# haoheliu/AudioLDM2

Measured on AMD Instinct MI355X. Metric: audio_seconds_per_second, higher is better.
Workload: dtype f32 storage/accumulate; each product = 6 bf16 MFMA partial products of exact 3-part operand splits (fp32-grade); 1 GPU; audioldm2-full: batch 8 prompts/GPU x 1 GPU, 10.24 s @16 kHz, 200 DDIM steps, CFG 3.5, eta 1.0, n_candidates 1; one step = sample_log + VAE decode + HiFi-GAN + D2H of the waveform; synthetic conditioning, random-init weights, host-CPU RNG noise; global_batch=8, parallelism=prompt-sharded replicas x1, weight_broadcast_bytes=0

## Files before the change

### audioldm2_amd/csrc/api.hip

```cpp
#include "common.h"
#include <string.h>

namespace aldm {
static thread_local char g_err[512] = "";
void set_error(const char* fmt, ...) {
    va_list ap;
    va_start(ap, fmt);
    vsnprintf(g_err, sizeof(g_err), fmt, ap);
    va_end(ap);
}
}

extern "C" int aldm_version(void) { return 25; }
extern "C" const char* aldm_last_error(void) { return aldm::g_err; }
```

### audioldm2_amd/csrc/igemm.hip

```cpp
#include "igemm_kernel.h"
#include <algorithm>
#include <atomic>
#include <stdlib.h>

namespace aldm {

int igemm_launch_pre0(int BM, int BN, int kgroups, bool uni, bool w8, dim3 grid, hipStream_t st, const IgemmK& p);
int igemm_launch_pre1(int BM, int BN, int kgroups, bool uni, bool w8, dim3 grid, hipStream_t st, const IgemmK& p);
int igemm_launch_pre2(int BM, int BN, int kgroups, bool uni, bool w8, dim3 grid, hipStream_t st, const IgemmK& p);
int igemm_launch_pre3(int BM, int BN, int kgroups, bool uni, bool w8, dim3 grid, hipStream_t st, const IgemmK& p);
int igemm_launch_pre4(int BM, int BN, int kgroups, bool uni, bool w8, dim3 grid, hipStream_t st, const IgemmK& p);
int igemm_launch_bx_pre0(int BM, int BN, int kgroups, bool uni, bool w8, dim3 grid, hipStream_t st, const IgemmK& p);
int igemm_launch_bx_pre1(int BM, int BN, int kgroups, bool uni, bool w8, dim3 grid, hipStream_t st, const IgemmK& p);
int igemm_launch_bx_pre2(int BM, int BN, int kgroups, bool uni, bool w8, dim3 grid, hipStream_t st, const IgemmK& p);
int igemm_launch_bx_pre3(int BM, int BN, int kgroups, bool uni, bool w8, dim3 grid, hipStream_t st, const IgemmK& p);

int igemm_launch_dma(int BM, int BN, int nst, int parts, bool f16, dim3 grid, hipStream_t st, const IgemmK& p);
bool igemm_dma_config_ok(int BM, int BN, int nst, int parts);
#ifdef ALDM_TEST_HOOKS
extern std::atomic<int> g_debug_drop_product;
#endif
int igemm_launch_dma_ws(int BM, int BN, int nst, int parts, int blocks, hipStream_t st, const IgemmK& p);
bool igemm_dma_ws_config_ok(int BM, int BN, int nst, int parts);
int igemm_dma_ws_blocks_per_cu(int BM, int BN, int nst, int parts);
// ... 22 lines not shown
    f32x4 v = *reinterpret_cast<const f32x4*>(w);
    int s = 1;
    for (; s + 3 < p.splits; s += 4) {
        const f32x4 a0 = *reinterpret_cast<const f32x4*>(w + (int64_t)s * slab);
        const f32x4 a1 = *reinterpret_cast<const f32x4*>(w + (int64_t)(s + 1) * slab);
        const f32x4 a2 = *reinterpret_cast<const f32x4*>(w + (int64_t)(s + 2) * slab);
        const f32x4 a3 = *reinterpret_cast<const f32x4*>(w + (int64_t)(s + 3) * slab);
        v += a0;
        v += a1;
        v += a2;
        v += a3;
    }
    for (; s < p.splits; ++s) v += *reinterpret_cast<const f32x4*>(w + (int64_t)s * slab);
    const int b = m / p.OHW;
    int64_t orow = m;
    if (d.out_mul > 0) {
        const int qq = m - b * p.OHW;
        const int t = qq * d.out_mul + d.out_off;
        if ((unsigned)t >= (unsigned)d.out_len) return;
        orow = (int64_t)b * d.out_len + t;
    }
    float* outp = d.out ? d.out + (int64_t)z * d.stride_o : nullptr;
    const float* resp = d.res ? d.res + (int64_t)z * d.stride_o : nullptr;
    const int64_t o = orow * d.ldo + n;
    f32x4 r;
#pragma unroll
    for (int j = 0; j < 4; ++j) r[j] = epi_value(d, p.rb_ld, outp, resp, b, o + j, n + j, v[j]);
    if (outp) {
#pragma unroll
        for (int j = 0; j < 4; ++j) outp[o + j] = r[j];
    }
    if (d.out_split) {
        if (d.out_split_act == ALDM_ACT_LRELU) {
#pragma unroll
            for (int j = 0; j < 4; ++j) r[j] = r[j] > 0.0f ? r[j] : r[j] * d.out_split_slope;
        }
// ... 3 lines not shown

__global__ void pack_weight_kernel(const float* __restrict__ src, float* __restrict__ dst, int N,
                                   int Cin, int KH, int KW, int Kg, int Npad) {
    const int64_t total = (int64_t)Kg * Npad * 4;
    for (int64_t i = blockIdx.x * (int64_t)blockDim.x + threadIdx.x; i < total;
         i += (int64_t)gridDim.x * blockDim.x) {
        const int j = i & 3;
        const int n = (i >> 2) % Npad;
        const int kg = (i >> 2) / Npad;
        const int k = kg * 4 + j;
        float v = 0.f;
        if (n < N && k < KH * KW * Cin) {
            const int tap = k / Cin, ci = k - tap * Cin;
            const int kh = tap / KW, kw = tap - kh * KW;
            v = src[(((int64_t)n * Cin + ci) * KH + kh) * KW + kw];
        }
        dst[i] = v;
    }
}

__global__ void pack_weight_tr_kernel(const float* __restrict__ src, float* __restrict__ dst, int N,
                                      int Cin, int KWfull, int T, int phase, int stride, int Kg,
                                      int Npad) {
    const int64_t total = (int64_t)Kg * Npad * 4;
    for (int64_t i = blockIdx.x * (int64_t)blockDim.x + threadIdx.x; i < total;
         i += (int64_t)gridDim.x * blockDim.x) {
        const int jj = i & 3;
        const int n = (i >> 2) % Npad;
        const int kg = (i >> 2) / Npad;
        const int k = kg * 4 + jj;
// ... 249 lines not shown
    ALDM_CHECK(d.SH > 0 && d.SW > 0 && d.DH > 0 && d.DW > 0, "aldm_igemm: bad stride/dilation");
    p.shh = log2_exact(d.up_h);
    p.shw = log2_exact(d.up_w);
    ALDM_CHECK(p.shh >= 0 && p.shw >= 0, "aldm_igemm: upsample factors must be powers of two");
    ALDM_CHECK((reinterpret_cast<uintptr_t>(d.x1) & 15) == 0 &&
                   (reinterpret_cast<uintptr_t>(d.w) & 15) == 0 &&
                   (d.x2 == nullptr || (reinterpret_cast<uintptr_t>(d.x2) & 15) == 0),
               "aldm_igemm: operands must be 16-byte aligned");
    if (d.b_mode == ALDM_B_NT) {
        ALDM_CHECK(d.ldb % 4 == 0 && d.ldb >= d.K, "aldm_igemm: NT ldb=%d invalid", d.ldb);
        p.Npad = d.N;
    } else {
        p.Npad = (d.N + 31) / 32 * 32;
        ALDM_CHECK(d.ldb == 0 || d.ldb == p.Npad, "aldm_igemm: packed ldb must equal Npad");
    }
    if (d.out_mul > 0) ALDM_CHECK(d.OH == 1, "aldm_igemm: row remap requires OH == 1");
    ALDM_CHECK((d.pre_scale == nullptr) == (d.pre_shift == nullptr),
               "aldm_igemm: pre_scale/pre_shift must come together");
    ALDM_CHECK(d.pre_scale == nullptr ||
                   ((reinterpret_cast<uintptr_t>(d.pre_scale) | reinterpret_cast<uintptr_t>(d.pre_shift)) & 15) == 0,
               "aldm_igemm: pre_scale/pre_shift must be 16-byte aligned");
    const bool geglu = d.epi_mode == ALDM_EPI_GEGLU;
    const bool qkv = d.epi_mode == ALDM_EPI_QKV;
    ALDM_CHECK(d.epi_mode == ALDM_EPI_PLAIN || geglu || qkv, "aldm_igemm: unknown epi_mode %d", d.epi_mode);
    if (qkv) {
        auto al16 = [](const void* q) { return (reinterpret_cast<uintptr_t>(q) & 15) == 0; };
        ALDM_CHECK(d.a_split && d.qkv_c > 0 && d.qkv_c % 64 == 0 && d.N == 3 * d.qkv_c && d.qkv_rows > 0 && d.qkv_rows % 32 == 0 &&
                       (((int64_t)d.B * d.OH * d.OW) % d.qkv_rows == 0 ||
                        d.qkv_rows == (((int64_t)d.B * d.OH * d.OW + 31) & ~(int64_t)31)) && d.out && d.k_split && d.vt_split && al16(d.out) &&
                       al16(d.k_split) && al16(d.vt_split) && d.ldo >= d.qkv_c && (d.ldo & 3) == 0 && !d.bias && !d.rowbias &&
                       !d.res && !d.out_split && !d.accumulate && d.out_mul == 0 && d.act == ALDM_ACT_NONE && d.alpha == 1.0f &&
// ... 35 lines not shown
        ALDM_CHECK(d.out_split_c > 0 && d.out_split_c % 32 == 0 && d.out_split_c >= (geglu ? d.N / 2 : d.N) &&
                       d.N % 4 == 0 && d.batch == 1 && (reinterpret_cast<uintptr_t>(d.out_split) & 15) == 0 &&
                       ((reinterpret_cast<uintptr_t>(d.out) | reinterpret_cast<uintptr_t>(d.res)) & 15) == 0 &&
                       (d.out == nullptr || (d.ldo & 3) == 0),
                   "aldm_igemm: out_split needs out_split_c %% 32 == 0 and >= N, N %% 4 == 0, batch 1, aligned out/res");
        ALDM_CHECK(d.out != nullptr || !d.accumulate, "aldm_igemm: accumulate needs an fp32 output");
    }
    if (d.a_split) {
        ALDM_CHECK(d.w_split != nullptr && d.b_mode == ALDM_B_PACKED && d.stride_w == 0 && d.batch == 1,
                   "aldm_igemm: a_split needs packed, split weights and batch 1");
        ALDM_CHECK(d.C2 == 0 && d.C1 % 32 == 0 && pre == PRE_NONE,
                   "aldm_igemm: a_split needs one source with C1 %% 32 == 0 and no prologue (C1=%d C2=%d)", d.C1, d.C2);
        ALDM_CHECK(((reinterpret_cast<uintptr_t>(d.a_split) | reinterpret_cast<uintptr_t>(d.w_split)) & 15) == 0,
                   "aldm_igemm: split images must be 16-byte aligned");
        ALDM_CHECK((int64_t)d.B * d.H * d.W * p.Cin * 2 * d.split_parts < (1ll << 40), "aldm_igemm: split image too large");
        const bool can_split = d.N % 4 == 0 && nk >= 8 && !geglu && !qkv;
        const bool have_ws = d.ws != nullptr && (reinterpret_cast<uintptr_t>(d.ws) & 15) == 0;
        auto dma_cost = [&](int bm, int bn, int nst, int sp, int* sp_eff) -> double {
            const int kt = cdiv(nk, sp);
            sp = cdiv(nk, kt);
            *sp_eff = sp;
            const double blocks = (double)cdiv64(Mz, bm) * cdiv(d.N, bn) * sp;
            const int lds = nst * (bm + bn) * 64 * d.split_parts;
            const int o = std::min(2, (160 * 1024) / lds);
            const double tile_c = (bm / 64) * (bn / 64) * 64.0 * (d.split_parts == 3 ? 6 : 3);
            const double dma_c = (bm + bn) * 64.0 * d.split_parts / 56.0;
            const double L = kt * std::max(tile_c, dma_c);
            const double one = kt * std::max(tile_c + 200.0, dma_c) + 6000.0;
            const int64_t nb = (int64_t)((blocks + 255.0) / 256.0);
            const int64_t full = nb / o, last = nb - full * o;
            double T = full * std::max(one, o * L);
            if (last) T += std::max(one, last * L);
            if (sp > 1) T += 10000.0 + (double)(sp + 1) * Mz * d.N * 4.0 / 2000.0;
            return T;
        };
        int splits = 1, nst = 0;
        const bool hint_fits = d.hint_bm > 0 && (!qkv || (d.hint_bn > 0 && d.qkv_c % d.hint_bn == 0)) && (!geglu || d.hint_bn == 128);
// ... 118 lines not shown
        p.tiles_n = cdiv(d.N, BN);
        p.kt_per_split = cdiv(nk, splits);
        splits = cdiv(nk, p.kt_per_split);
        if (splits > 1 && (!have_ws || d.ws_floats < (int64_t)splits * p.M * d.N)) {
            splits = 1;
            p.kt_per_split = nk;
        }
        p.splits = splits;
        p.kgroups = 1;
        p.bx = 1;
        p.pre = pre;
        p.dma = 1;
        p.nst = nst;
        p.ws = 0;
        p.ws_blocks = 0;
        if (lw_nst > 0) {
            ALDM_CHECK(igemm_dma_lw_config_ok(BM, BN, lw_nst, d.split_parts), "aldm_igemm: no loader-wave DMA kernel for tile %dx%d, %d stages", BM, BN, lw_nst);
            p.ws = 2;
            p.nst = lw_nst;
        }
        if (ws_nst > 0) {
            if (splits == 1 && d.a_fmt == ALDM_FMT_BF16 && d.out_split_parts == d.split_parts && d.out_split_fmt == ALDM_FMT_BF16 &&
                igemm_dma_ws_config_ok(BM, BN, ws_nst, d.split_parts) && dma_ws_eligible(p, BM, BN)) {
                const int ntiles = p.tiles_m * p.tiles_n;
                const int per = cdiv(ntiles, device_cus() * igemm_dma_ws_blocks_per_cu(BM, BN, ws_nst, d.split_parts));
                p.ws = 1;
                p.nst = ws_nst;
                p.ws_blocks = cdiv(ntiles, per);
            } else {
                ALDM_CHECK(!g_force_bm, "aldm_igemm: the persistent DMA kernel cannot run this launch (tile %dx%d, %d stages)", BM,
// ... 93 lines not shown
    p.splits = splits;
    p.kgroups = kgroups;
    p.bx = bx_ok && BN != 32 ? 1 : 0;
    p.pre = pre;
    return 0;
}

extern "C" int aldm_igemm_plan(const aldm_igemm_desc* dd, int* bm, int* bn, int64_t* flops, int* splits,
                               int* kgroups, int* mma) {
    IgemmK p;
    int BM, BN;
    const int rc = igemm_prepare(dd, p, BM, BN);
    if (rc) return rc;
    if (bm) *bm = BM;
    if (bn) *bn = BN;
    if (flops) *flops = 2ll * p.M * p.d.N * p.d.K * p.d.batch;
    if (splits) *splits = p.splits;
    if (kgroups) *kgroups = p.kgroups;
    if (mma) *mma = p.bx ? ALDM_MMA_BF16X6 : ALDM_MMA_F32;
    return 0;
}

extern "C" int aldm_igemm_plan_stages(const aldm_igemm_desc* dd) {
    IgemmK p;
    int BM, BN;
    if (igemm_prepare(dd, p, BM, BN)) return -1;
    if (p.dma && p.ws == 4) return 400 + (BM == 128 && p.ws_blocks == 4 ? 10 : 0) + p.nst;
    return p.dma ? p.nst + 100 * p.ws : 0;
}

extern "C" int aldm_igemm_plan_epilogue(const aldm_igemm_desc* dd) {
// ... 9 lines not shown
    t.ws = reinterpret_cast<float*>(uintptr_t(16));
    t.ws_floats = INT64_MAX;
    IgemmK p;
    int BM, BN;
    if (igemm_prepare(&t, p, BM, BN)) return 0;
    return p.splits > 1 ? (int64_t)p.d.batch * p.splits * p.M * p.d.N : 0;
}

extern "C" int aldm_igemm(const aldm_igemm_desc* dd, void* stream) {
    IgemmK p;
    int BM, BN;
    int rc = igemm_prepare(dd, p, BM, BN);
    if (rc) return rc;
    p.epi_form = plan_epilogue_form(p, BM, BN);
    const aldm_igemm_desc& d = p.d;
    dim3 grid((unsigned)(p.tiles_m * p.tiles_n), (unsigned)p.splits, (unsigned)d.batch);
    hipStream_t st = (hipStream_t)stream;
    const int pre = p.pre;
    const bool uni = p.OHW % BM == 0;
    const int env_w8 = g_wave8_mask < 0 ? default_wave8_mask() : g_wave8_mask;
    const bool gn_pre = pre == PRE_AFFINE || pre == PRE_AFFINE_SILU;
    const int tile_bit = (BM == 128 && BN == 128) ? 1 : (BM == 64 && BN == 128) ? 2 : (BM == 128 && BN == 64) ? 4 : 0;
    const bool w8 = p.kgroups == 1 && d.epi_mode != ALDM_EPI_GEGLU && (env_w8 & tile_bit) != 0 &&
                    (p.bx ? tile_bit == 1 : (gn_pre || (tile_bit == 1 && (env_w8 & 8) != 0)));
#ifdef ALDM_TEST_HOOKS
    if (g_debug_drop_product.load(std::memory_order_relaxed))
        ALDM_CHECK(p.dma && p.ws == 0 && BM == 64 && BN == 128 && p.nst == 2 && d.split_parts == 3,
                   "aldm_igemm: aldm_debug_drop_product is set: force the classic DMA-fed 64x128 tile with 2 stages and 3-part images "
                   "(got dma=%d form=%d tile %dx%d, %d stages, %d parts) or clear the switch", p.dma, p.ws, BM, BN, p.nst, d.split_parts);
#endif
    if (p.dma && p.ws == 4) {
// ... 93 lines not shown
    } else {
        ALDM_CHECK(KH == 1 && stride > 0 && phase >= 0 && phase < stride,
                   "aldm_pack_weight: bad transposed args");
        const int T = (KW + stride - 1) / stride;
        const int K = T * Cin;
        const int Kg = (K + 3) / 4;
        const int64_t total = (int64_t)Kg * Npad * 4;
        const int blocks = (int)std::min<int64_t>(cdiv64(total, 256), 4096);
        hipLaunchKernelGGL(pack_weight_tr_kernel, dim3(blocks), dim3(256), 0, st, src, dst, N, Cin,
                           KW, T, phase, stride, Kg, Npad);
    }
    ALDM_LAUNCH_CHECK("aldm_pack_weight");
    return 0;
}

extern "C" int aldm_pack_kn(const float* src, float* dst, int K, int N, int lds, int batch,
                            int64_t stride_src, int64_t stride_dst, void* stream) {
    ALDM_CHECK(src && dst && K > 0 && N > 0 && lds >= N && batch > 0, "aldm_pack_kn: bad args");
    const int Npad = (N + 31) / 32 * 32;
    const int Kg = (K + 3) / 4;
    const int64_t total = (int64_t)Kg * Npad * 4;
    const int blocks = (int)std::min<int64_t>(cdiv64(total, 256), 4096);
    hipLaunchKernelGGL(pack_kn_kernel, dim3(blocks, batch), dim3(256), 0, (hipStream_t)stream, src,
                       dst, K, N, lds, Kg, Npad, stride_src, stride_dst);
    ALDM_LAUNCH_CHECK("aldm_pack_kn");
    return 0;
}
```

### audioldm2_amd/csrc/igemm_dma.h

```cpp
#pragma once
#include "igemm_epilogue.h"
#include <type_traits>

namespace aldm {

static __device__ __attribute__((aligned(256))) unsigned g_dma_zero_page[256 + 64];

constexpr int dma_stage_slots(int BM, int BN, int NP) { return (BM + BN) * 4 * NP; }
constexpr int dma_lds_bytes(int BM, int BN, int NST, int NP) { return NST * dma_stage_slots(BM, BN, NP) * 16; }
constexpr int dma_blocks_per_cu(int BM, int BN, int NST, int NP) {
    return (160 * 1024) / dma_lds_bytes(BM, BN, NST, NP) >= 2 ? 2 : 1;
}

template <bool F16>
__device__ __forceinline__ f32x16 mfma_32x32x16(const bf16x8 a, const bf16x8 b, const f32x16 c) {
    if constexpr (F16)
        return __builtin_amdgcn_mfma_f32_32x32x16_f16(__builtin_bit_cast(f16x8, a), __builtin_bit_cast(f16x8, b), c, 0, 0, 0);
    else
        return __builtin_amdgcn_mfma_f32_32x32x16_bf16(a, b, c, 0, 0, 0);
}
template <bool F16, int MT, int NT>
__device__ __forceinline__ void unscale_acc(f32x16 (&acc)[MT][NT], float acc_scale) {
    if constexpr (F16) {
#pragma unroll
// ... 53 lines not shown
        tile_m = logical / p.tiles_n;
    }
    const int m0 = tile_m * BM, n0 = tile_n * BN;
    const int split = blockIdx.y;
    const int nk_all = d.K >> 5;
    const int kt0 = split * p.kt_per_split;
    const int kt1 = min(nk_all, kt0 + p.kt_per_split);
#if ALDM_DMA_ABLATE & 32
    const int nk = min(kt1 - kt0, 1);
#else
    const int nk = kt1 - kt0;
#endif

    const char* zero = reinterpret_cast<const char*>(g_dma_zero_page);
    const char* abase = reinterpret_cast<const char*>(d.a_split);
    const char* wbase = reinterpret_cast<const char*>(d.w_split);
    const int cpb = p.Cin >> 5;
    const int taps = d.KH * d.KW;
    const int64_t rowbytes = (int64_t)cpb * PB;

    const int lane_off = ((lane & 3) ^ ((lane >> 4) & 3)) * 16;
    int a_pix[RA], a_h[RA], a_w[RA];
#pragma unroll
    for (int i = 0; i < RA; ++i) {
        const int m = m0 + (wave * RA + i) * 16 + (lane >> 2);
        if (m < p.M) {
            const int b = m / p.OHW;
            const int rem = m - b * p.OHW;
            const int oh = rem / d.OW;
            const int ow = rem - oh * d.OW;
            a_pix[i] = b * d.H;
            a_h[i] = oh * d.SH - d.PH;
            a_w[i] = ow * d.SW - d.PW;
        } else {
            a_pix[i] = 0;
            a_h[i] = -(1 << 28);
            a_w[i] = 0;
        }
    }
    const char* a_ptr[RA];
    int a_step[RA];
    int t_kh, t_kw, t_cb;
    auto set_tap = [&]() {
        const int dh = t_kh * d.DH, dw = t_kw * d.DW;
        const int cboff = t_cb * PB + lane_off;
#pragma unroll
        for (int i = 0; i < RA; ++i) {
            const int ihv = a_h[i] + dh, iwv = a_w[i] + dw;
// ... 203 lines not shown
#if ALDM_DMA_ABLATE & 16
    if (p.M == -12345) {
#pragma unroll
        for (int i = 0; i < MT; ++i)
#pragma unroll
            for (int j = 0; j < NT; ++j)
#pragma unroll
                for (int e = 0; e < 16; ++e) d.ws[(i * NT + j) * 16 + e + threadIdx.x * 256] = acc[i][j][e];
    }
    return;
#endif
    unscale_acc<F16>(acc, d.acc_scale);
    if constexpr (FORM != ALDM_EPI_FORM_GENERIC)
        igemm_epilogue_form<MT, NT, NP, FORM>(p, acc, epre, reinterpret_cast<float*>(&smem[0]), m0, n0, wave, wm, wn, lane);
    else
        igemm_epilogue<MT, NT>(p, acc, reinterpret_cast<float*>(&smem[0]), m0, n0, wave, wm, wn, lane, 0, split);
}

}
```

### audioldm2_amd/csrc/igemm_epilogue.h

```cpp
#pragma once
#include "common.h"

#ifndef ALDM_DMA_ABLATE
#define ALDM_DMA_ABLATE 0
#endif

namespace aldm {

struct IgemmK {
    aldm_igemm_desc d;
    int Cin, M, OHW, HV, WV, shh, shw, Kg, Npad, tiles_m, tiles_n;
    int splits, kt_per_split;
    int kgroups;
    int rb_ld;
    int bx;
    int pre;
    int dma;
    int nst;
    int ws;
    int ws_blocks;
    int os_rows;
    int epi_form;
};

// ... 111 lines not shown
}
__device__ __forceinline__ void split_store4_out(const aldm_igemm_desc& d, void* img, int64_t row, int Cs, int c, const f32x4 v) {
    if (d.out_split_fmt == ALDM_FMT_F16) split_store4_f16(img, row, Cs, c, v, d.out_split_scale);
    else split_store4(img, row, Cs, c, v, d.out_split_parts);
}

template <int P>
__device__ __forceinline__ void split_store4_t(void* img, int64_t row, int Cs, int c, const f32x4 v) {
    static_assert(P == 2 || P == 3, "2 or 3 parts");
    u32x2 part[3];
    if constexpr (P == 2) split4_rn2(v, part);
    else split4(v, part);
    char* base = reinterpret_cast<char*>(img) + (row * (Cs >> 5) + (c >> 5)) * (64 * P) + (c & 31) * 2;
#pragma unroll
    for (int q = 0; q < P; ++q) *reinterpret_cast<u32x2*>(base + q * 64) = part[q];
}

__device__ __forceinline__ float epi_value(const aldm_igemm_desc& d, int rb_ld, const float* __restrict__ outp,
                                           const float* __restrict__ resp, int b, int64_t o, int n, float v) {
    if (d.bias) v += d.bias[n];
    if (d.rowbias) v += d.rowbias[(int64_t)b * rb_ld + n];
    v = act_apply(v, d.act, d.act_slope);
    if (resp) v += resp[o];
    v *= d.alpha;
    if (d.accumulate) v += outp[o];
    return v;
}

__device__ __forceinline__ float silu_fast(float v) {
    return v * __frcp_rn(1.0f + __expf(-v));
// ... 138 lines not shown
        f32x4 v[ITC];
        int64_t rowoff[ITC];
        int64_t srow[ITC];
        int rboff[ITC];
        unsigned okmask = 0;
#pragma unroll
        for (int it = 0; it < ITC; ++it) {
            const int r = (itc + it) * RPI + sr;
            v[it] = *reinterpret_cast<const f32x4*>(&stg[r * SP + sc]);
            const int m = m0 + (wm * MT + i) * 32 + r;
            bool ok = m < p.M && ncol < d.N;
            int b = 0;
            int64_t orow = m;
            if (need_b) {
                b = m / p.OHW;
                if (d.out_mul > 0) {
                    const int qq = m - b * p.OHW;
                    const int t = qq * d.out_mul + d.out_off;
                    ok = ok && (unsigned)t < (unsigned)d.out_len;
                    orow = (int64_t)b * d.out_len + t;
                }
            }
            rowoff[it] = ok ? orow * ld_out + (ncol - col_shift) : 0;
            srow[it] = orow;
            rboff[it] = ok ? b * p.rb_ld + ncol : 0;
            okmask |= ((ok && epi_st) ? 1u : 0u) << it;
        }
        if (split_out) {
#pragma unroll
            for (int it = 0; it < ITC; ++it)
                if ((okmask >> it) & 1u) *reinterpret_cast<f32x4*>(outp + rowoff[it]) = v[it];
            continue;
        }
#pragma unroll
        for (int it = 0; it < ITC; ++it) v[it] += bias4;
        if (d.rowbias) {
// ... 181 lines not shown
```

### audioldm2_amd/lib.py

```python
from __future__ import annotations

import ctypes as C
import os

_HERE = os.path.dirname(os.path.abspath(__file__))
LIB_PATH = os.environ.get("ALDM_LIB_PATH") or os.path.join(_HERE, "libaldm_hip.so")
ABI_VERSION = 25

ACT_NONE, ACT_SILU, ACT_LRELU, ACT_TANH, ACT_LOGCLAMP, ACT_GELU, ACT_GELU_TANH = range(7)
B_PACKED, B_NT = 0, 1
EPI_PLAIN, EPI_GEGLU, EPI_QKV = 0, 1, 2
GN_CHUNKED, GN_FUSED, GN_FUSED_SPLIT = 0, 1, 2
FMT_BF16, FMT_F16 = 0, 1
EPI_FORM_GENERIC, EPI_FORM_PLAIN, EPI_FORM_ROWBIAS, EPI_FORM_RES = range(4)


class IgemmDesc(C.Structure):

    _fields_ = [
        ("x1", C.c_void_p), ("x2", C.c_void_p),
        ("C1", C.c_int32), ("C2", C.c_int32),
        ("pix1", C.c_int32), ("pix2", C.c_int32),
        ("B", C.c_int32), ("H", C.c_int32), ("W", C.c_int32),
        ("up_h", C.c_int32), ("up_w", C.c_int32),
# ... 8 lines not shown
        ("bias", C.c_void_p), ("rowbias", C.c_void_p), ("res", C.c_void_p), ("out", C.c_void_p),
        ("ldo", C.c_int32), ("act", C.c_int32), ("act_slope", C.c_float), ("alpha", C.c_float),
        ("accumulate", C.c_int32),
        ("out_mul", C.c_int32), ("out_off", C.c_int32), ("out_len", C.c_int32),
        ("batch", C.c_int32),
        ("stride_x", C.c_int64), ("stride_w", C.c_int64), ("stride_o", C.c_int64),
        ("rowbias_ld", C.c_int32), ("epi_mode", C.c_int32),
        ("ws", C.c_void_p), ("ws_floats", C.c_int64),
        ("hint_bm", C.c_int32), ("hint_bn", C.c_int32), ("hint_splits", C.c_int32), ("hint_kgroups", C.c_int32),
        ("w_split", C.c_void_p), ("hint_mma", C.c_int32), ("hint_stages", C.c_int32),
        ("a_split", C.c_void_p), ("out_split", C.c_void_p), ("out_split_c", C.c_int32), ("split_parts", C.c_int32),
        ("out_split_act", C.c_int32), ("out_split_slope", C.c_float),
        ("k_split", C.c_void_p), ("vt_split", C.c_void_p), ("qkv_c", C.c_int32), ("qkv_rows", C.c_int32),
        ("a_fmt", C.c_int32), ("acc_scale", C.c_float), ("out_split_parts", C.c_int32),
        ("out_split_fmt", C.c_int32), ("out_split_scale", C.c_float), ("vt_scale", C.c_float),
    ]


MAX_WINDOWS = 32


class WindowStarts(C.Structure):

    _fields_ = [("n", C.c_int), ("s", C.c_int * MAX_WINDOWS)]


MAX_ROWS = 64


class WindowRows(C.Structure):
# ... 28 lines not shown
    "aldm_split_bytes_parts": (C.c_int64, [C.c_int, C.c_int, C.c_int]),
    "aldm_pack_split_bf16_parts": (C.c_int, [C.c_void_p, C.c_void_p, C.c_int, C.c_int, C.c_int, C.c_void_p]),
    "aldm_pack_split_f16": (C.c_int, [C.c_void_p, C.c_void_p, C.c_int, C.c_int, C.c_float, C.c_void_p]),
    "aldm_split_rows_f16": (C.c_int, [C.c_void_p, C.c_void_p, C.c_int, C.c_int, C.c_int64, C.c_int, C.c_void_p, C.c_void_p,
                                      C.c_int, C.c_float, C.c_void_p, C.c_void_p, C.c_int, C.c_float, C.c_void_p]),
    "aldm_groupnorm_split_f16": (C.c_int, [C.c_void_p, C.c_void_p, C.c_int, C.c_int, C.c_int, C.c_int, C.c_int, C.c_float,
                                           C.c_void_p, C.c_void_p, C.c_int, C.c_void_p, C.c_void_p, C.c_void_p, C.c_void_p,
                                           C.c_void_p, C.c_int, C.c_float, C.c_void_p]),
    "aldm_layernorm_split_f16": (C.c_int, [C.c_void_p, C.c_void_p, C.c_void_p, C.c_int, C.c_int, C.c_void_p, C.c_void_p,
                                           C.c_float, C.c_float, C.c_void_p]),
    "aldm_igemm_mma": (C.c_int, [C.c_int]),
    "aldm_split_bytes": (C.c_int64, [C.c_int, C.c_int]),
    "aldm_pack_split_bf16": (C.c_int, [C.c_void_p, C.c_void_p, C.c_int, C.c_int, C.c_void_p]),
    "aldm_pack_weight": (C.c_int, [C.c_void_p, C.c_void_p, C.c_int, C.c_int, C.c_int, C.c_int,
                                   C.c_int, C.c_int, C.c_int, C.c_void_p]),
    "aldm_pack_kn": (C.c_int, [C.c_void_p, C.c_void_p, C.c_int, C.c_int, C.c_int, C.c_int,
                               C.c_int64, C.c_int64, C.c_void_p]),
    "aldm_groupnorm_stats": (C.c_int, [C.c_void_p, C.c_void_p, C.c_int, C.c_int, C.c_int, C.c_int,
                                       C.c_int, C.c_float, C.c_void_p, C.c_void_p, C.c_void_p,
                                       C.c_void_p, C.c_void_p, C.c_void_p]),
    "aldm_gn_ws_floats": (C.c_int64, [C.c_int, C.c_int, C.c_int, C.c_int]),
    "aldm_groupnorm_plan": (C.c_int, [C.c_int] * 6 + [C.POINTER(C.c_int)] * 9),
    "aldm_groupnorm_split": (C.c_int, [C.c_void_p, C.c_void_p, C.c_int, C.c_int, C.c_int, C.c_int, C.c_int, C.c_float,
                                       C.c_void_p, C.c_void_p, C.c_int, C.c_void_p, C.c_void_p, C.c_void_p, C.c_void_p,
                                       C.c_void_p, C.c_int, C.c_void_p]),
    "aldm_layernorm": (C.c_int, [C.c_void_p, C.c_void_p, C.c_int, C.c_int, C.c_void_p, C.c_void_p,
                                 C.c_float, C.c_void_p]),
    "aldm_attention_mma": (C.c_int, [C.c_int]),
    "aldm_attention_sched": (C.c_int, [C.c_int]),
    "aldm_attention_query_tiles": (C.c_int, [C.c_int, C.c_int, C.c_int]),
# ... 177 lines not shown
```

### audioldm2_amd/ops.py

```python
from __future__ import annotations

import ctypes as C
import json
import os
from dataclasses import dataclass
from typing import List, Optional, Sequence, Tuple

import torch

from . import lib as _l
from .lib import (ACT_GELU, ACT_GELU_TANH, ACT_LOGCLAMP, ACT_LRELU, ACT_NONE, ACT_SILU, ACT_TANH, B_NT, B_PACKED,
                  IgemmDesc)


def _stream() -> int:
    return torch.cuda.current_stream().cuda_stream


def _p(t: Optional[torch.Tensor]):
    return None if t is None else t.data_ptr()


def _chk(t: torch.Tensor, name: str):
    if not (t.is_cuda and t.dtype == torch.float32 and t.is_contiguous()):
# ... 467 lines not shown
def pack_conv(weight: torch.Tensor, bias: Optional[torch.Tensor] = None) -> Packed:
    w = weight.detach().to(device="cuda", dtype=torch.float32).contiguous()
    if w.dim() == 2:
        N, Cin, KH, KW = w.shape[0], w.shape[1], 1, 1
    elif w.dim() == 3:
        N, Cin, KH, KW = w.shape[0], w.shape[1], 1, w.shape[2]
    else:
        N, Cin, KH, KW = w.shape
    K = KH * KW * Cin
    dst = torch.empty(((K + 3) // 4) * _npad(N) * 4, device="cuda", dtype=torch.float32)
    lib = _l.load()
    _l.check(lib.aldm_pack_weight(w.data_ptr(), dst.data_ptr(), N, Cin, KH, KW, 0, 0, 1, _stream()),
             "pack_weight")
    b = None if bias is None else bias.detach().to(device="cuda", dtype=torch.float32).contiguous()
    return Packed(dst, N, Cin, KH, KW, b)


def pack_geglu(weight: torch.Tensor, bias: Optional[torch.Tensor]) -> Packed:
    two_inner = weight.shape[0]
    inner = two_inner // 2
    assert weight.dim() == 2 and two_inner % 64 == 0
    g = torch.arange(inner // 32).view(-1, 1, 1)
    j = torch.arange(2).view(1, -1, 1)
    l = torch.arange(32).view(1, 1, -1)
    perm = (j * inner + g * 32 + l).reshape(-1).to(weight.device)
    pw = pack_conv(weight.detach()[perm], None if bias is None else bias.detach()[perm])
    pw.geglu = True
    return pw


# ... 145 lines not shown
    for ph in range(stride):
        dst = torch.empty(((T * Cin + 3) // 4) * _npad(N) * 4, device="cuda", dtype=torch.float32)
        _l.check(lib.aldm_pack_weight(w.data_ptr(), dst.data_ptr(), N, Cin, 1, KW, 1, ph, stride,
                                      _stream()), "pack_weight(tr)")
        out.append(Packed(dst, N, Cin, 1, T, b))
    return out


def conv(x: torch.Tensor, pw: Packed, *, stride=(1, 1), pad=(0, 0), dil=(1, 1), up=(1, 1),
         x2: Optional[torch.Tensor] = None, out_hw: Optional[Tuple[int, int]] = None,
         pre: Optional[Tuple[torch.Tensor, torch.Tensor]] = None, pre_act: int = ACT_NONE,
         pre_slope: float = 0.0, bias: Optional[torch.Tensor] = None,
         rowbias: Optional[torch.Tensor] = None, res: Optional[torch.Tensor] = None,
         act: int = ACT_NONE, act_slope: float = 0.0, alpha: float = 1.0,
         out: Optional[torch.Tensor] = None, accumulate: bool = False,
         remap: Optional[Tuple[int, int, int]] = None,
         use_pw_bias: bool = True, split_out: Optional[str] = None, split_act: int = ACT_NONE, split_slope: float = 0.0):
    is_split = isinstance(x, SplitT)
    if is_split:
        assert x2 is None and pre is None and pre_act == ACT_NONE, "a pre-split operand takes no prologue"
    else:
        _chk(x, "conv.x")
    B, H, W, C1 = x.shape
    C2 = 0
    if x2 is not None:
        _chk(x2, "conv.x2")
        assert x2.shape[:3] == x.shape[:3]
        C2 = x2.shape[3]
    assert C1 + C2 == pw.Cin, f"channels {C1}+{C2} != packed Cin {pw.Cin}"
    VH, VW = H * up[0], W * up[1]
    if out_hw is None:
        OH = (VH + 2 * pad[0] - dil[0] * (pw.KH - 1) - 1) // stride[0] + 1
        OW = (VW + 2 * pad[1] - dil[1] * (pw.KW - 1) - 1) // stride[1] + 1
    else:
        OH, OW = out_hw
    N = pw.N
    if remap is not None:
        out_mul, out_off, out_len = remap
        oshape = (B, 1, out_len, N)
    else:
        out_mul = out_off = out_len = 0
        oshape = (B, OH, OW, N)
    if split_out == "only":
        assert out is None and not accumulate
    elif out is None:
        assert not accumulate
        out = torch.empty(oshape, device=x.device, dtype=torch.float32)
    else:
        _chk(out, "conv.out")
        assert out.numel() == oshape[0] * oshape[1] * oshape[2] * oshape[3], (out.shape, oshape)
    so = SplitT.empty(oshape, x.device) if split_out else None
    if bias is None and use_pw_bias:
# ... 15 lines not shown
    d.w = pw.data.data_ptr(); d.b_mode = B_PACKED; d.ldb = 0
    if not is_split:
        d.w_split = pw.split_ptr(3)
    d.K = pw.K; d.N = N
    d.bias = _p(bias); d.rowbias = _p(rowbias); d.res = _p(res); d.out = _p(out)
    if so is not None:
        d.out_split = so.data_ptr(); d.out_split_c = N
        d.out_split_act = split_act; d.out_split_slope = split_slope
    if rowbias is not None:
        if not (rowbias.dim() == 2 and rowbias.stride(1) == 1 and rowbias.shape == (B, N)):
            raise RuntimeError("conv.rowbias: need a [B, N] fp32 view with unit inner stride")
        d.rowbias_ld = rowbias.stride(0)
    d.ldo = N; d.act = act; d.act_slope = act_slope; d.alpha = alpha
    d.accumulate = 1 if accumulate else 0
    d.out_mul = out_mul; d.out_off = out_off; d.out_len = out_len
    d.batch = 1
    _igemm(d, "igemm(conv)")
    if split_out == "only":
        return so
    return (out.view(oshape), so) if split_out else out.view(oshape)


def linear(x, pw: Packed, **kw):
    shp = x.shape
    if isinstance(x, SplitT):
        M = x.rows
        y = conv(x.view(1, 1, M, shp[-1]), pw, **kw)
    else:
        M = x.numel() // shp[-1]
        y = conv(x.reshape(1, 1, M, shp[-1]), pw, **kw)
# ... 982 lines not shown
```

### audioldm2_amd/unet.py

```python
from __future__ import annotations

from typing import List, Optional

import torch
import torch.nn as nn

import os

from . import ops
from .ops import ACT_NONE, ACT_SILU

PRESPLIT_ATTENTION = os.environ.get("ALDM_ATTN_PRESPLIT", "1") != "0" and "ALDM_ATTN_MMA" not in os.environ


class ResBlock(nn.Module):

    def __init__(self, channels, emb_channels, dropout, out_channels=None):
        super().__init__()
        self.channels = channels
        self.out_channels = out_channels or channels
        self.in_layers = nn.Sequential(nn.GroupNorm(32, channels), nn.SiLU(),
                                       nn.Conv2d(channels, self.out_channels, 3, padding=1))
        self.emb_layers = nn.Sequential(nn.SiLU(), nn.Linear(emb_channels, self.out_channels))
        self.out_layers = nn.Sequential(nn.GroupNorm(32, self.out_channels), nn.SiLU(), nn.Dropout(p=dropout),
# ... 58 lines not shown
            self._pk = ops.pack_conv(self.op.weight, self.op.bias)
        if ops.use_dma() and self.channels % 32 == 0:
            x = ops.split_rows(x)
        return ops.conv(x, self._pk, stride=(2, 2), pad=(1, 1))


class Upsample(nn.Module):

    def __init__(self, channels, use_conv=True, dims=2, out_channels=None, padding=1):
        super().__init__()
        assert use_conv and dims == 2
        self.channels = channels
        self.out_channels = out_channels or channels
        self.conv = nn.Conv2d(channels, self.out_channels, 3, padding=padding)
        self._pk = None

    def run(self, x):
        if self._pk is None:
            self._pk = ops.pack_conv(self.conv.weight, self.conv.bias)
        if ops.use_dma() and self.channels % 32 == 0:
            x = ops.split_rows(x)
        return ops.conv(x, self._pk, pad=(1, 1), up=(2, 2))


class GEGLU(nn.Module):
    def __init__(self, dim_in, dim_out):
        super().__init__()
        self.proj = nn.Linear(dim_in, dim_out * 2)


class FeedForward(nn.Module):

    def __init__(self, dim, mult=4, dropout=0.0):
        super().__init__()
        self.net = nn.Sequential(GEGLU(dim, dim * mult), nn.Dropout(dropout), nn.Linear(dim * mult, dim))

# ... 400 lines not shown
```

### include/aldm_hip.h

```cpp
#ifndef ALDM_HIP_H
#define ALDM_HIP_H

#include <stdint.h>

#ifdef __cplusplus
extern "C" {
#endif

int aldm_version(void);
const char* aldm_last_error(void);

enum {
    ALDM_ACT_NONE = 0,
    ALDM_ACT_SILU = 1,
    ALDM_ACT_LRELU = 2,
    ALDM_ACT_TANH = 3,
    ALDM_ACT_LOGCLAMP = 4,
    ALDM_ACT_GELU = 5,
    ALDM_ACT_GELU_TANH = 6
};

enum { ALDM_EPI_PLAIN = 0, ALDM_EPI_GEGLU = 1, ALDM_EPI_QKV = 2 };

enum {
// ... 45 lines not shown
    void* out_split;
    int32_t out_split_c;
    int32_t split_parts;
    int32_t out_split_act;
    float out_split_slope;
    void* k_split;
    void* vt_split;
    int32_t qkv_c;
    int32_t qkv_rows;
    int32_t a_fmt;
    float acc_scale;
    int32_t out_split_parts;
    int32_t out_split_fmt;
    float out_split_scale;
    float vt_scale;
} aldm_igemm_desc;

int aldm_igemm(const aldm_igemm_desc* d, void* stream);
int64_t aldm_igemm_ws_floats(const aldm_igemm_desc* d);
enum { ALDM_FMT_BF16 = 0, ALDM_FMT_F16 = 1 };
int aldm_igemm_plan(const aldm_igemm_desc* d, int* bm, int* bn, int64_t* flops, int* splits, int* kgroups,
                    int* mma);
int aldm_igemm_plan_stages(const aldm_igemm_desc* d);
enum { ALDM_EPI_FORM_GENERIC = 0, ALDM_EPI_FORM_PLAIN = 1, ALDM_EPI_FORM_ROWBIAS = 2, ALDM_EPI_FORM_RES = 3 };
int aldm_igemm_plan_epilogue(const aldm_igemm_desc* d);
int aldm_igemm_epilogue_forms(int on);
void aldm_igemm_force(int bm, int bn, int splits, int kgroups);
void aldm_igemm_force_stages(int stages);
int aldm_igemm_wave8_mask(int mask);
int aldm_igemm_mma(int mode);
// ... 5 lines not shown
int64_t aldm_split_bytes_parts(int K, int N, int parts);
int aldm_pack_split_bf16_parts(const float* packed, void* dst, int K, int N, int parts, void* stream);
int aldm_pack_split_f16(const float* packed, void* dst, int K, int N, float scale, void* stream);

int64_t aldm_split_image_bytes(int64_t rows, int C, int parts);
int aldm_split_rows(const float* x1, const float* x2, int C1, int C2, int64_t rows, int P, const float* scale,
                    const float* shift, int act, void* dst, void* dst_raw, int parts, void* stream);
int aldm_split_rows_act(const float* x1, const float* x2, int C1, int C2, int64_t rows, int P, const float* scale,
                        const float* shift, int act, float slope, void* dst, void* dst_raw, int parts, void* stream);
int aldm_split_rows_f16(const float* x1, const float* x2, int C1, int C2, int64_t rows, int P, const float* scale,
                        const float* shift, int act, float slope, void* dst, void* dst_raw, int raw_parts, float f16_scale,
                        void* stream);

int aldm_pack_weight(const float* src, float* dst, int N, int Cin, int KH, int KW,
                     int transposed, int phase, int stride, void* stream);
int aldm_pack_kn(const float* src, float* dst, int K, int N, int lds, int batch,
                 int64_t stride_src, int64_t stride_dst, void* stream);

int aldm_groupnorm_stats(const float* x1, const float* x2, int B, int P, int C1, int C2,
                         int G, float eps, const float* gamma, const float* beta,
                         float* scale, float* shift, float* ws, void* stream);
int64_t aldm_gn_ws_floats(int B, int P, int C, int G);
enum { ALDM_GN_CHUNKED = 0, ALDM_GN_FUSED = 1, ALDM_GN_FUSED_SPLIT = 2 };
int aldm_groupnorm_plan(int B, int P, int C1, int C2, int G, int want_split, int* form, int* group_slices,
                        int* groups_per_block, int* chunks, int* chunk_px, int* cols, int* rows, int* passes,
                        int* active_threads);
int aldm_groupnorm_split(const float* x1, const float* x2, int B, int P, int C1, int C2, int G, float eps,
                         const float* gamma, const float* beta, int act, float* scale, float* shift, float* ws,
                         void* dst, void* dst_raw, int parts, void* stream);
int aldm_groupnorm_split_f16(const float* x1, const float* x2, int B, int P, int C1, int C2, int G, float eps,
// ... 146 lines not shown
```

Before: 19.22 audio-s/s.

## Fold nearest-2x upsample into 3x3 conv as four phased 2x2 convolutions

```diff
diff --git a/audioldm2_amd/csrc/api.hip b/audioldm2_amd/csrc/api.hip
--- a/audioldm2_amd/csrc/api.hip
+++ b/audioldm2_amd/csrc/api.hip
@@ -11,5 +11,5 @@
 }
 }
 
-extern "C" int aldm_version(void) { return 25; }
+extern "C" int aldm_version(void) { return 26; }
 extern "C" const char* aldm_last_error(void) { return aldm::g_err; }
diff --git a/audioldm2_amd/csrc/igemm.hip b/audioldm2_amd/csrc/igemm.hip
--- a/audioldm2_amd/csrc/igemm.hip
+++ b/audioldm2_amd/csrc/igemm.hip
@@ -60,12 +60,7 @@
     for (; s < p.splits; ++s) v += *reinterpret_cast<const f32x4*>(w + (int64_t)s * slab);
     const int b = m / p.OHW;
     int64_t orow = m;
-    if (d.out_mul > 0) {
-        const int qq = m - b * p.OHW;
-        const int t = qq * d.out_mul + d.out_off;
-        if ((unsigned)t >= (unsigned)d.out_len) return;
-        orow = (int64_t)b * d.out_len + t;
-    }
+    if (d.out_mul > 0 && !epi_remap_row(d, b, m - b * p.OHW, orow)) return;
     float* outp = d.out ? d.out + (int64_t)z * d.stride_o : nullptr;
     const float* resp = d.res ? d.res + (int64_t)z * d.stride_o : nullptr;
     const int64_t o = orow * d.ldo + n;
@@ -99,6 +94,32 @@
             const int tap = k / Cin, ci = k - tap * Cin;
             const int kh = tap / KW, kw = tap - kh * KW;
             v = src[(((int64_t)n * Cin + ci) * KH + kh) * KW + kw];
+        }
+        dst[i] = v;
+    }
+}
+
+__global__ void pack_upfold2_kernel(const float* __restrict__ src, float* __restrict__ dst, int N, int Cin, int Kg, int Npad) {
+    const int64_t slab = (int64_t)Kg * Npad * 4;
+    const int64_t total = 4 * slab;
+    for (int64_t i = blockIdx.x * (int64_t)blockDim.x + threadIdx.x; i < total; i += (int64_t)gridDim.x * blockDim.x) {
+        const int ph = (int)(i / slab);
+        const int64_t r = i - ph * slab;
+        const int j = r & 3;
+        const int n = (r >> 2) % Npad;
+        const int kg = (r >> 2) / Npad;
+        const int k = kg * 4 + j;
+        float v = 0.f;
+        if (n < N && k < 4 * Cin) {
+            const int tap = k / Cin, ci = k - tap * Cin;
+            const int a = ph >> 1, b = ph & 1, ty = tap >> 1, tx = tap & 1;
+            const int y0 = ty == 0 ? 0 : 2 - (1 - a), y1 = ty == 0 ? a : 2;
+            const int x0 = tx == 0 ? 0 : 2 - (1 - b), x1 = tx == 0 ? b : 2;
+            const float* w = src + ((int64_t)n * Cin + ci) * 9;
+            double s = 0.0;
+            for (int ky = y0; ky <= y1; ++ky)
+                for (int kx = x0; kx <= x1; ++kx) s += (double)w[ky * 3 + kx];
+            v = (float)s;
         }
         dst[i] = v;
     }
@@ -378,7 +399,20 @@
         p.Npad = (d.N + 31) / 32 * 32;
         ALDM_CHECK(d.ldb == 0 || d.ldb == p.Npad, "aldm_igemm: packed ldb must equal Npad");
     }
-    if (d.out_mul > 0) ALDM_CHECK(d.OH == 1, "aldm_igemm: row remap requires OH == 1");
+    ALDM_CHECK(d.out_mul_h >= 0 && (d.out_mul_h == 0 || d.out_mul > 0), "aldm_igemm: out_mul_h needs out_mul > 0");
+    if (d.out_mul_h > 0)
+        ALDM_CHECK(d.out_off >= 0 && d.out_off < d.out_mul && d.out_off_h >= 0 && d.out_off_h < d.out_mul_h &&
+                       (int64_t)d.out_mul * d.OW == d.out_len && (int64_t)d.B * d.OH * d.out_mul_h * d.out_len < (1ll << 31),
+                   "aldm_igemm: 2-D row remap needs 0 <= out_off < out_mul, 0 <= out_off_h < out_mul_h, out_len == out_mul * OW");
+    else if (d.out_mul > 0)
+        ALDM_CHECK(d.OH == 1, "aldm_igemm: row remap requires OH == 1");
+    if (d.out_phases == 1) d.out_phases = 0;
+    if (d.out_phases != 0)
+        ALDM_CHECK(d.out_phases == 4 && d.out_mul_h == 2 && d.out_mul == 2 && d.out_off == 0 && d.out_off_h == 0 && d.a_split &&
+                       d.batch <= 1 && d.stride_o == 0 && d.PH >= 1 && d.PW >= 1 && d.w_split_phase_bytes > 0 &&
+                       (d.w_split_phase_bytes & 15) == 0 && d.epi_mode == ALDM_EPI_PLAIN,
+                   "aldm_igemm: out_phases must be 0 or 4, with the 2-D remap (2, 0, 2, 0), PH, PW >= 1, a pre-split operand, batch 1, "
+                   "the plain epilogue and a 16-byte aligned w_split_phase_bytes");
     ALDM_CHECK((d.pre_scale == nullptr) == (d.pre_shift == nullptr),
                "aldm_igemm: pre_scale/pre_shift must come together");
     ALDM_CHECK(d.pre_scale == nullptr ||
@@ -444,13 +478,14 @@
         ALDM_CHECK(((reinterpret_cast<uintptr_t>(d.a_split) | reinterpret_cast<uintptr_t>(d.w_split)) & 15) == 0,
                    "aldm_igemm: split images must be 16-byte aligned");
         ALDM_CHECK((int64_t)d.B * d.H * d.W * p.Cin * 2 * d.split_parts < (1ll << 40), "aldm_igemm: split image too large");
-        const bool can_split = d.N % 4 == 0 && nk >= 8 && !geglu && !qkv;
+        const int phases = d.out_phases > 1 ? d.out_phases : 1;
+        const bool can_split = d.N % 4 == 0 && nk >= 8 && !geglu && !qkv && phases == 1;
         const bool have_ws = d.ws != nullptr && (reinterpret_cast<uintptr_t>(d.ws) & 15) == 0;
         auto dma_cost = [&](int bm, int bn, int nst, int sp, int* sp_eff) -> double {
             const int kt = cdiv(nk, sp);
             sp = cdiv(nk, kt);
             *sp_eff = sp;
-            const double blocks = (double)cdiv64(Mz, bm) * cdiv(d.N, bn) * sp;
+            const double blocks = (double)cdiv64(Mz, bm) * cdiv(d.N, bn) * sp * phases;
             const int lds = nst * (bm + bn) * 64 * d.split_parts;
             const int o = std::min(2, (160 * 1024) / lds);
             const double tile_c = (bm / 64) * (bn / 64) * 64.0 * (d.split_parts == 3 ? 6 : 3);
@@ -599,6 +634,8 @@
         p.nst = nst;
         p.ws = 0;
         p.ws_blocks = 0;
+        ALDM_CHECK(phases == 1 || (lw_nst == 0 && ws_nst == 0 && splits == 1),
+                   "aldm_igemm: a phased launch (out_phases) runs on the classic DMA-fed kernel without split-K only");
         if (lw_nst > 0) {
             ALDM_CHECK(igemm_dma_lw_config_ok(BM, BN, lw_nst, d.split_parts), "aldm_igemm: no loader-wave DMA kernel for tile %dx%d, %d stages", BM, BN, lw_nst);
             p.ws = 2;
@@ -722,7 +759,7 @@
     if (rc) return rc;
     if (bm) *bm = BM;
     if (bn) *bn = BN;
-    if (flops) *flops = 2ll * p.M * p.d.N * p.d.K * p.d.batch;
+    if (flops) *flops = 2ll * p.M * p.d.N * p.d.K * p.d.batch * (p.d.out_phases > 1 ? p.d.out_phases : 1);
     if (splits) *splits = p.splits;
     if (kgroups) *kgroups = p.kgroups;
     if (mma) *mma = p.bx ? ALDM_MMA_BF16X6 : ALDM_MMA_F32;
@@ -762,7 +799,7 @@
     if (rc) return rc;
     p.epi_form = plan_epilogue_form(p, BM, BN);
     const aldm_igemm_desc& d = p.d;
-    dim3 grid((unsigned)(p.tiles_m * p.tiles_n), (unsigned)p.splits, (unsigned)d.batch);
+    dim3 grid((unsigned)(p.tiles_m * p.tiles_n), (unsigned)p.splits, (unsigned)(d.out_phases > 1 ? d.out_phases : d.batch));
     hipStream_t st = (hipStream_t)stream;
     const int pre = p.pre;
     const bool uni = p.OHW % BM == 0;
@@ -886,6 +923,17 @@
     return 0;
 }
 
+extern "C" int aldm_pack_upfold2(const float* src, float* dst, int N, int Cin, void* stream) {
+    ALDM_CHECK(src && dst && N > 0 && Cin > 0, "aldm_pack_upfold2: bad args");
+    const int Npad = (N + 31) / 32 * 32;
+    const int Kg = Cin;
+    const int64_t total = 4ll * Kg * Npad * 4;
+    const int blocks = (int)std::min<int64_t>(cdiv64(total, 256), 4096);
+    hipLaunchKernelGGL(pack_upfold2_kernel, dim3(blocks), dim3(256), 0, (hipStream_t)stream, src, dst, N, Cin, Kg, Npad);
+    ALDM_LAUNCH_CHECK("aldm_pack_upfold2");
+    return 0;
+}
+
 extern "C" int aldm_pack_kn(const float* src, float* dst, int K, int N, int lds, int batch,
                             int64_t stride_src, int64_t stride_dst, void* stream) {
     ALDM_CHECK(src && dst && K > 0 && N > 0 && lds >= N && batch > 0, "aldm_pack_kn: bad args");
diff --git a/audioldm2_amd/csrc/igemm_dma.h b/audioldm2_amd/csrc/igemm_dma.h
--- a/audioldm2_amd/csrc/igemm_dma.h
+++ b/audioldm2_amd/csrc/igemm_dma.h
@@ -91,7 +91,9 @@
 
     const char* zero = reinterpret_cast<const char*>(g_dma_zero_page);
     const char* abase = reinterpret_cast<const char*>(d.a_split);
-    const char* wbase = reinterpret_cast<const char*>(d.w_split);
+    const int phase = __builtin_amdgcn_readfirstlane(blockIdx.z);
+    const int pad_h = d.PH - (phase >> 1), pad_w = d.PW - (phase & 1);
+    const char* wbase = reinterpret_cast<const char*>(d.w_split) + (int64_t)phase * d.w_split_phase_bytes;
     const int cpb = p.Cin >> 5;
     const int taps = d.KH * d.KW;
     const int64_t rowbytes = (int64_t)cpb * PB;
@@ -107,8 +109,8 @@
             const int oh = rem / d.OW;
             const int ow = rem - oh * d.OW;
             a_pix[i] = b * d.H;
-            a_h[i] = oh * d.SH - d.PH;
-            a_w[i] = ow * d.SW - d.PW;
+            a_h[i] = oh * d.SH - pad_h;
+            a_w[i] = ow * d.SW - pad_w;
         } else {
             a_pix[i] = 0;
             a_h[i] = -(1 << 28);
@@ -342,7 +344,7 @@
     if constexpr (FORM != ALDM_EPI_FORM_GENERIC)
         igemm_epilogue_form<MT, NT, NP, FORM>(p, acc, epre, reinterpret_cast<float*>(&smem[0]), m0, n0, wave, wm, wn, lane);
     else
-        igemm_epilogue<MT, NT>(p, acc, reinterpret_cast<float*>(&smem[0]), m0, n0, wave, wm, wn, lane, 0, split);
-}
-
-}
+        igemm_epilogue<MT, NT>(p, acc, reinterpret_cast<float*>(&smem[0]), m0, n0, wave, wm, wn, lane, phase, split);
+}
+
+}
diff --git a/audioldm2_amd/csrc/igemm_epilogue.h b/audioldm2_amd/csrc/igemm_epilogue.h
--- a/audioldm2_amd/csrc/igemm_epilogue.h
+++ b/audioldm2_amd/csrc/igemm_epilogue.h
@@ -149,6 +149,18 @@
     char* base = reinterpret_cast<char*>(img) + (row * (Cs >> 5) + (c >> 5)) * (64 * P) + (c & 31) * 2;
 #pragma unroll
     for (int q = 0; q < P; ++q) *reinterpret_cast<u32x2*>(base + q * 64) = part[q];
+}
+
+__device__ __forceinline__ bool epi_remap_row(const aldm_igemm_desc& d, int b, int qq, int64_t& orow, int phase = 0) {
+    if (d.out_mul_h > 0) {
+        const int oh = qq / d.OW, ow = qq - oh * d.OW;
+        orow = ((int64_t)b * (d.OH * d.out_mul_h) + (oh * d.out_mul_h + d.out_off_h + (phase >> 1))) * d.out_len +
+               (ow * d.out_mul + d.out_off + (phase & 1));
+        return true;
+    }
+    const int t = qq * d.out_mul + d.out_off;
+    orow = (int64_t)b * d.out_len + t;
+    return (unsigned)t < (unsigned)d.out_len;
 }
 
 __device__ __forceinline__ float epi_value(const aldm_igemm_desc& d, int rb_ld, const float* __restrict__ outp,
@@ -317,12 +329,7 @@
             int64_t orow = m;
             if (need_b) {
                 b = m / p.OHW;
-                if (d.out_mul > 0) {
-                    const int qq = m - b * p.OHW;
-                    const int t = qq * d.out_mul + d.out_off;
-                    ok = ok && (unsigned)t < (unsigned)d.out_len;
-                    orow = (int64_t)b * d.out_len + t;
-                }
+                if (d.out_mul > 0) ok = epi_remap_row(d, b, m - b * p.OHW, orow, d.out_phases > 1 ? z : 0) && ok;
             }
             rowoff[it] = ok ? orow * ld_out + (ncol - col_shift) : 0;
             srow[it] = orow;
diff --git a/audioldm2_amd/csrc/upfold.hip b/audioldm2_amd/csrc/upfold.hip
--- /dev/null
+++ b/audioldm2_amd/csrc/upfold.hip
@@ -0,0 +1,12 @@
+#include "common.h"
+
+static constexpr int64_t UPFOLD_MIN_PHASE_ROWS = 4096;
+static constexpr int64_t UPFOLD_ONE_LAUNCH_MAX_ROWS = INT64_MAX;
+
+extern "C" int aldm_upfold_plan(int B, int H, int W, int C, int N) {
+    if (B < 1 || H < 1 || W < 1 || C < 32 || C % 32 != 0 || N < 1) return 0;
+    if ((int64_t)B * H * W * 4 >= (1ll << 31) - 256) return 0;
+    const int64_t rows = (int64_t)B * H * W;
+    if (rows < UPFOLD_MIN_PHASE_ROWS) return 1;
+    return rows <= UPFOLD_ONE_LAUNCH_MAX_ROWS ? 3 : 2;
+}
diff --git a/audioldm2_amd/lib.py b/audioldm2_amd/lib.py
--- a/audioldm2_amd/lib.py
+++ b/audioldm2_amd/lib.py
@@ -5,7 +5,7 @@
 
 _HERE = os.path.dirname(os.path.abspath(__file__))
 LIB_PATH = os.environ.get("ALDM_LIB_PATH") or os.path.join(_HERE, "libaldm_hip.so")
-ABI_VERSION = 25
+ABI_VERSION = 26
 
 ACT_NONE, ACT_SILU, ACT_LRELU, ACT_TANH, ACT_LOGCLAMP, ACT_GELU, ACT_GELU_TANH = range(7)
 B_PACKED, B_NT = 0, 1
@@ -46,6 +46,8 @@
         ("k_split", C.c_void_p), ("vt_split", C.c_void_p), ("qkv_c", C.c_int32), ("qkv_rows", C.c_int32),
         ("a_fmt", C.c_int32), ("acc_scale", C.c_float), ("out_split_parts", C.c_int32),
         ("out_split_fmt", C.c_int32), ("out_split_scale", C.c_float), ("vt_scale", C.c_float),
+        ("out_mul_h", C.c_int32), ("out_off_h", C.c_int32),
+        ("out_phases", C.c_int32), ("w_split_phase_bytes", C.c_int64),
     ]
 
 
@@ -104,6 +106,8 @@
     "aldm_pack_split_bf16": (C.c_int, [C.c_void_p, C.c_void_p, C.c_int, C.c_int, C.c_void_p]),
     "aldm_pack_weight": (C.c_int, [C.c_void_p, C.c_void_p, C.c_int, C.c_int, C.c_int, C.c_int,
                                    C.c_int, C.c_int, C.c_int, C.c_void_p]),
+    "aldm_pack_upfold2": (C.c_int, [C.c_void_p, C.c_void_p, C.c_int, C.c_int, C.c_void_p]),
+    "aldm_upfold_plan": (C.c_int, [C.c_int] * 5),
     "aldm_pack_kn": (C.c_int, [C.c_void_p, C.c_void_p, C.c_int, C.c_int, C.c_int, C.c_int,
                                C.c_int64, C.c_int64, C.c_void_p]),
     "aldm_groupnorm_stats": (C.c_int, [C.c_void_p, C.c_void_p, C.c_int, C.c_int, C.c_int, C.c_int,
diff --git a/audioldm2_amd/ops.py b/audioldm2_amd/ops.py
--- a/audioldm2_amd/ops.py
+++ b/audioldm2_amd/ops.py
@@ -505,6 +505,101 @@
              "pack_weight")
     b = None if bias is None else bias.detach().to(device="cuda", dtype=torch.float32).contiguous()
     return Packed(dst, N, Cin, KH, KW, b)
+
+
+def _parse_switch(v):
+    v = "1" if v is None else str(v).strip()
+    if v in ("0", "False"):
+        return False
+    if v in ("", "1", "True"):
+        return True
+    return frozenset(int(t) for t in v.split(",") if t.strip())
+
+
+UPFOLD = _parse_switch(os.environ.get("ALDM_UPFOLD"))
+
+
+class PackedUpfold2:
+
+    def __init__(self, data: torch.Tensor, N: int, Cin: int, bias: Optional[torch.Tensor]):
+        self.data = data
+        self.N, self.Cin, self.bias = N, Cin, bias
+        self._pk = [Packed(data[ph], N, Cin, 2, 2, bias) for ph in range(4)]
+        self._img = {}
+
+    def phases(self, parts: int) -> List[Packed]:
+        if parts not in self._img:
+            if torch.cuda.is_current_stream_capturing():
+                raise RuntimeError("a folded weight's split image must exist before graph capture (run one eager step)")
+            lib = _l.load()
+            K = 4 * self.Cin
+            img = torch.empty((4, lib.aldm_split_bytes_parts(K, self.N, parts) // 4), device=self.data.device, dtype=torch.int32)
+            for ph in range(4):
+                _l.check(lib.aldm_pack_split_bf16_parts(self.data[ph].data_ptr(), img[ph].data_ptr(), K, self.N, parts, _stream()),
+                         "pack_split_bf16(upfold2)")
+                if parts == 2:
+                    self._pk[ph].split2 = img[ph]
+                else:
+                    self._pk[ph].split = img[ph]
+            self._img[parts] = img
+        return self._pk
+
+    def phase_bytes(self, parts: int) -> int:
+        return self._img[parts].stride(0) * 4
+
+
+def pack_conv_upfold2(weight: torch.Tensor, bias: Optional[torch.Tensor] = None) -> PackedUpfold2:
+    w = weight.detach().to(device="cuda", dtype=torch.float32).contiguous()
+    assert w.dim() == 4 and w.shape[2:] == (3, 3), w.shape
+    N, Cin = w.shape[:2]
+    dst = torch.empty((4, Cin * _npad(N) * 4), device="cuda", dtype=torch.float32)
+    _l.check(_l.load().aldm_pack_upfold2(w.data_ptr(), dst.data_ptr(), N, Cin, _stream()), "pack_upfold2")
+    b = None if bias is None else bias.detach().to(device="cuda", dtype=torch.float32).contiguous()
+    return PackedUpfold2(dst, N, Cin, b)
+
+
+def upfold(on=None):
+    global UPFOLD
+    prev = UPFOLD
+    if on is not None:
+        UPFOLD = on if isinstance(on, bool) else frozenset(int(c) for c in on)
+    return prev
+
+
+def upfold_plan(B: int, H: int, W: int, C: int, N: int) -> dict:
+    rc = _l.load().aldm_upfold_plan(B, H, W, C, N)
+    return {"supported": rc >= 1, "use": rc >= 2, "one_launch": rc == 3}
+
+
+UPFOLD_FORM = {"1": True, "4": False}.get(os.environ.get("ALDM_UPFOLD_FORM", ""))
+
+
+def upfold_applies(B: int, H: int, W: int, C: int, N: int) -> bool:
+    if not use_dma() or UPFOLD is False:
+        return False
+    plan = upfold_plan(B, H, W, C, N)
+    if UPFOLD is True:
+        return plan["use"]
+    return plan["supported"] and C in UPFOLD
+
+
+def conv_upfold2(x: "SplitT", pf: PackedUpfold2, out: Optional[torch.Tensor] = None,
+                 one_launch: Optional[bool] = None) -> torch.Tensor:
+    assert isinstance(x, SplitT) and x.fmt == "bf16"
+    B, H, W, C = x.shape
+    assert C == pf.Cin
+    if out is None:
+        out = torch.empty((B, 2 * H, 2 * W, pf.N), device=x.device, dtype=torch.float32)
+    if one_launch is None:
+        one_launch = UPFOLD_FORM if UPFOLD_FORM is not None else upfold_plan(B, H, W, C, pf.N)["one_launch"]
+    if one_launch:
+        pw = pf.phases(x.parts)[0]
+        conv(x, pw, pad=(1, 1), out_hw=(H, W), remap2d=(2, 0, 2, 0), out=out, phase_bytes=pf.phase_bytes(x.parts))
+        return out.view(B, 2 * H, 2 * W, pf.N)
+    for ph, pw in enumerate(pf.phases(x.parts)):
+        a, b = ph >> 1, ph & 1
+        conv(x, pw, pad=(1 - a, 1 - b), out_hw=(H, W), remap2d=(2, a, 2, b), out=out)
+    return out.view(B, 2 * H, 2 * W, pf.N)
 
 
 def pack_geglu(weight: torch.Tensor, bias: Optional[torch.Tensor]) -> Packed:
@@ -680,8 +775,8 @@
          rowbias: Optional[torch.Tensor] = None, res: Optional[torch.Tensor] = None,
          act: int = ACT_NONE, act_slope: float = 0.0, alpha: float = 1.0,
          out: Optional[torch.Tensor] = None, accumulate: bool = False,
-         remap: Optional[Tuple[int, int, int]] = None,
-         use_pw_bias: bool = True, split_out: Optional[str] = None, split_act: int = ACT_NONE, split_slope: float = 0.0):
+         remap: Optional[Tuple[int, int, int]] = None, remap2d: Optional[Tuple[int, int, int, int]] = None,
+         phase_bytes: int = 0, use_pw_bias: bool = True, split_out: Optional[str] = None, split_act: int = ACT_NONE, split_slope: float = 0.0):
     is_split = isinstance(x, SplitT)
     if is_split:
         assert x2 is None and pre is None and pre_act == ACT_NONE, "a pre-split operand takes no prologue"
@@ -701,7 +796,13 @@
     else:
         OH, OW = out_hw
     N = pw.N
-    if remap is not None:
+    out_mul_h = out_off_h = 0
+    if remap2d is not None:
+        assert remap is None
+        out_mul_h, out_off_h, out_mul, out_off = remap2d
+        out_len = out_mul * OW
+        oshape = (B, OH * out_mul_h, out_len, N)
+    elif remap is not None:
         out_mul, out_off, out_len = remap
         oshape = (B, 1, out_len, N)
     else:
@@ -747,6 +848,10 @@
     d.ldo = N; d.act = act; d.act_slope = act_slope; d.alpha = alpha
     d.accumulate = 1 if accumulate else 0
     d.out_mul = out_mul; d.out_off = out_off; d.out_len = out_len
+    d.out_mul_h = out_mul_h; d.out_off_h = out_off_h
+    if phase_bytes:
+        assert is_split and remap2d == (2, 0, 2, 0)
+        d.out_phases = 4; d.w_split_phase_bytes = phase_bytes
     d.batch = 1
     _igemm(d, "igemm(conv)")
     if split_out == "only":
diff --git a/audioldm2_amd/unet.py b/audioldm2_amd/unet.py
--- a/audioldm2_amd/unet.py
+++ b/audioldm2_amd/unet.py
@@ -96,12 +96,19 @@
         self.out_channels = out_channels or channels
         self.conv = nn.Conv2d(channels, self.out_channels, 3, padding=padding)
         self._pk = None
+        self._pf = None
 
     def run(self, x):
         if self._pk is None:
             self._pk = ops.pack_conv(self.conv.weight, self.conv.bias)
         if ops.use_dma() and self.channels % 32 == 0:
+            B, H, W, C = x.shape
+            fold = ops.upfold_applies(B, H, W, C, self.out_channels)
             x = ops.split_rows(x)
+            if fold:
+                if self._pf is None:
+                    self._pf = ops.pack_conv_upfold2(self.conv.weight, self.conv.bias)
+                return ops.conv_upfold2(x, self._pf)
         return ops.conv(x, self._pk, pad=(1, 1), up=(2, 2))
 
 
diff --git a/include/aldm_hip.h b/include/aldm_hip.h
--- a/include/aldm_hip.h
+++ b/include/aldm_hip.h
@@ -83,6 +83,9 @@
     int32_t out_split_fmt;
     float out_split_scale;
     float vt_scale;
+    int32_t out_mul_h, out_off_h;
+    int32_t out_phases;
+    int64_t w_split_phase_bytes;
 } aldm_igemm_desc;
 
 int aldm_igemm(const aldm_igemm_desc* d, void* stream);
@@ -118,6 +121,8 @@
 
 int aldm_pack_weight(const float* src, float* dst, int N, int Cin, int KH, int KW,
                      int transposed, int phase, int stride, void* stream);
+int aldm_pack_upfold2(const float* src, float* dst, int N, int Cin, void* stream);
+int aldm_upfold_plan(int B, int H, int W, int C, int N);
 int aldm_pack_kn(const float* src, float* dst, int K, int N, int lds, int batch,
                  int64_t stride_src, int64_t stride_dst, void* stream);
 
```

New measurement: 19.39 audio-s/s (median of 6 runs). Within noise of the previous version (+0.9%).
